# DanHelmy/hdr-realtime-video-pipeline

Hardware: AMD Instinct MI355X
Metric: frames/sec (HDRTVNet++ AGCM+LE+HG fp16 3840x2160 + fused RGB48 post into the pinned host ring); p50 per-frame ms in p50_ms (higher is better)
Workload: dtype f16

## Files before the change

hdr-realtime-video-pipeline_amd/csrc/api_graph.hip:

```cpp
#include "api.h"

namespace hdrtv_host {

void Seq::conv(const std::string &key, const f16 *src0, int c0, const f16 *src1, int c1, int Hi, int Wi, int act, int mode, f16 *dst, int dstC, int Hd, int Wd, const f16 *res1, const f16 *res2, f16 *dst_full, f16 *dst_planar, const f16 *res_planar, const float *dotw, float *dst_dot, int s0_stride)
{
    if (!ok()) return;
    auto it = c->conv.find(key);
    if (it == c->conv.end()) { rc = fail(c, HDRTV_ESTATE, "no packed conv %s", key.c_str()); return; }
    const ConvLayer &L = it->second;
    ConvParams p;
    memset(&p, 0, sizeof p);
    p.src0 = src0; p.src1 = src1; p.c0 = c0; p.c1 = c1;
    p.s0_stride = s0_stride ? s0_stride : c0; p.s1_stride = c1;
    p.Hi = Hi; p.Wi = Wi;
    const int pad = L.ks / 2;
    p.Ho = (Hi + 2 * pad - L.ks) / L.stride + 1;
    p.Wo = (Wi + 2 * pad - L.ks) / L.stride + 1;
    p.wpk = wtp<f16>(c, L.wpk); p.scale = wtp<float>(c, L.scale); p.shift = wtp<float>(c, L.shift);
    p.CoutPad = L.coutPad; p.Cout = L.cout; p.act = act; p.mode = mode;
    p.dst = dst; p.dst_full = dst_full; p.dstC = dstC; p.Hd = Hd; p.Wd = Wd;
    p.res1 = res1; p.res2 = res2; p.dst_planar = dst_planar; p.res_planar = res_planar;
    p.dotw = dotw; p.dst_dot = dst_dot;
    if (c0 + c1 != L.cin) { rc = fail(c, HDRTV_ESTATE, "conv %s: channel mismatch", key.c_str()); return; }
    p.zeros = wtp<f16>(c, c->zeros_off);
// ... 247 lines not shown
            snprintf(b, sizeof b, "cls%d.g", i - 1); ng = wtp<float>(c, c->f32v.at(b));
            snprintf(b, sizeof b, "cls%d.be", i - 1); nb = wtp<float>(c, c->f32v.at(b));
        }
        snprintf(b, sizeof b, "cls%d.w", i);
        const float *w = wtp<float>(c, c->f32v.at(b));
        snprintf(b, sizeof b, "cls%d.b", i);
        const float *bias = wtp<float>(c, c->f32v.at(b));
        int nblk = 0;
        q.chk(cls_block_launch(in, i == 0, cls_ci[i], s.ch[i], s.cw[i], nm, nr, ng, nb, w, bias, cls_co[i], out, s.ch[i + 1],
                               s.cw[i + 1], q.wsp<float>("agcm.part"), q.s, c->cls_q[i].on ? &c->cls_q[i] : nullptr,
                               (i == 4 && c->cls_q[5].on) ? &c->cls_q[5] : nullptr, &nblk),
              "cls_block", c->cls_q[i].on ? "cls_block<fq>" : "cls_block", (double)s.ch[i] * s.cw[i] * cls_ci[i] * cls_co[i]);
        snprintf(a, sizeof a, "agcm.mean%d", i + 1);
        snprintf(b, sizeof b, "agcm.rstd%d", i + 1);
        q.chk(cls_stats_launch(q.wsp<float>("agcm.part"), cls_co[i], nblk, s.ch[i + 1] * s.cw[i + 1], 1e-5f, q.wsp<float>(a),
                               q.wsp<float>(b), q.s),
              "cls_stats", "cls_stats");
    }
    AgcmFoldArgs fa;
    fa.mean5 = q.wsp<float>("agcm.mean5");
    fa.w20 = wtp<float>(c, c->f32v.at("cls20.w")); fa.b20 = wtp<float>(c, c->f32v.at("cls20.b"));
    for (int st = 0; st < 3; ++st) {
        snprintf(a, sizeof a, "gfm.s%d.w", st); fa.ws[st] = wtp<float>(c, c->f32v.at(a));
        snprintf(a, sizeof a, "gfm.s%d.b", st); fa.bs[st] = wtp<float>(c, c->f32v.at(a));
        snprintf(a, sizeof a, "gfm.t%d.w", st); fa.wt[st] = wtp<float>(c, c->f32v.at(a));
        snprintf(a, sizeof a, "gfm.t%d.b", st); fa.bt[st] = wtp<float>(c, c->f32v.at(a));
    }
    fa.w1 = wtp<float>(c, c->f32v.at("agcm.w1")); fa.b1 = wtp<float>(c, c->f32v.at("agcm.b1"));
    fa.w2 = wtp<float>(c, c->f32v.at("agcm.w2")); fa.b2 = wtp<float>(c, c->f32v.at("agcm.b2"));
    fa.w3 = wtp<float>(c, c->f32v.at("agcm.w3")); fa.b3 = wtp<float>(c, c->f32v.at("agcm.b3"));
    if (c->agcm_q8) {
        AgcmFoldQ8Args qa;
        qa.q20 = c->cls_q[5];
        for (int i = 0; i < 6; ++i) qa.qlin[i] = c->lin_q[i];
        qa.P = wtp<float>(c, c->ag_P); qa.Q = wtp<float>(c, c->ag_Q);
        qa.inv2 = c->ag_q[1].inv(); qa.inv3 = c->ag_q[2].inv();
        qa.consts = q.wsp<float>("agcm.qconst");
        q.chk(agcm_fold_q8_launch(fa, qa, q.wsp<float>("agcm.bias"), q.s), "agcm_fold", "agcm_fold<q8>", 128.0 * 6 + 6.0 * (64 + 64 + 3) * 2);
        q.chk(agcm_mlp_q8_launch(rgb, agcm_out, (size_t)c->H * c->W, wtp<int8_t>(c, c->ag_frag), qa.consts, c->ag_q[0].inv(), c->ag_q[0].zoff(),
                                 c->ag_q[1].zoff(), c->ag_q[2].zoff(), q.s),
              "agcm_mlp", "agcm_mlp<q8>", (double)c->H * c->W * (3 * 64 + 64 * 64 + 64 * 3), 12.0 * c->H * c->W);
        return q.rc;
    }
    q.chk(agcm_fold_launch(fa, q.wsp<f16>("agcm.frags"), q.wsp<float>("agcm.bias"), q.s), "agcm_fold", "agcm_fold",
          128.0 * 6 + 6.0 * (64 + 64 + 3) * 2);
    q.chk(agcm_mlp_launch(rgb, agcm_out, (size_t)c->H * c->W, q.wsp<f16>("agcm.frags"), q.wsp<float>("agcm.bias"), q.s),
          "agcm_mlp", "agcm_mlp", (double)c->H * c->W * (3 * 64 + 64 * 64 + 64 * 3), 12.0 * c->H * c->W);
    return q.rc;
}

int run_le(hdrtv_ctx *c, Seq &q, const f16 *img, f16 *out_planar)
{
    const Shapes s = shapes_for(c->H, c->W);
    const int H = s.H, W = s.W;
    f16 *cond = q.wsp<f16>("le.cond");
    f16 *cond1 = q.wsp<f16>("le.cond1"), *cond2 = q.wsp<f16>("le.cond2"), *cond3 = q.wsp<f16>("le.cond3"),
        *cond4 = q.wsp<f16>("le.cond4");
    f16 *h2a = q.wsp<f16>("le.h2a");
    auto qlast = [&](const QLastLayer &Q, QLastArgs &a) -> const QLastArgs * {
        if (!Q.on) return nullptr;
        a.wq = wtp<int8_t>(c, Q.wq); a.ss = wtp<float>(c, Q.ss); a.q_inv = Q.q.inv(); a.q_zoff = Q.q.zoff();
        return &a;
    };
    QLastArgs qa6, qa2;
    if (q.ok() && c->trunk_q8) {
        TrunkQ8Args ta;
        ta.wfrag = wtp<int8_t>(c, c->tq_frag); ta.consts = wtp<float>(c, c->tq_const);
        ta.q1_inv = c->tq_q[0].inv(); ta.q1_zoff = c->tq_q[0].zoff(); ta.q4_inv = c->tq_q[3].inv();
        for (int i = 0; i < 5; ++i) ta.zoff[i] = c->tq_q[i + 1].zoff();
        q.chk(le_cond_trunk_q8_launch(img, H, W, ta, cond, cond1, c->n_cu, q.s), "LE.cond_trunk", "le_cond_trunk_q8",
              (double)H * W * (27 * 64 + 4 * 64 * 64 + 64 * 16), (double)H * W * (6 + 128 + 32));
    } else if (q.ok())
        q.chk(le_cond_trunk_launch(img, H, W, wtp<f16>(c, c->trunk_wfrag), wtp<float>(c, c->trunk_bias), cond, cond1, c->n_cu, q.s,
                                   qlast(c->q_trunk6, qa6)),
              "LE.cond_trunk", c->q_trunk6.on ? "le_cond_trunk<q6>" : "le_cond_trunk", (double)H * W * (27 * 64 + 4 * 64 * 64 + 64 * 16), (double)H * W * (6 + 128 + 32));
    auto isq8 = [&](const char *L) { return c->q8.find(L) != c->q8.end(); };
    auto qof = [&](const char *L) -> const ActQf * { auto it = c->q8.find(L); return it == c->q8.end() ? nullptr : &it->second.q; };
    f16 *h2b = q.wsp<f16>("le.h2b");
    const f16 *a2 = nullptr, *a3 = nullptr, *a4 = nullptr;
    const int8_t *a2q = nullptr, *a3q = nullptr, *a4q = nullptr;
    int astride = 64;
    bool cond2_fused = false;
    if (c->conv.find("LE.CondNet234.0") != c->conv.end()) {
        f16 *x192 = q.wsp<f16>("le.x192");
        cond2_fused = c->var.at("cond2_fused") != 0 && !c->tail_q8 && !c->q_tail2.on;
        if (cond2_fused) { q.tail_w = wtp<f16>(c, c->tail_wfrag); q.tail_b = wtp<float>(c, c->tail_bias); q.tail_out = cond2; }
        q.conv("LE.CondNet234.0", cond, 64, nullptr, 0, H, W, ACT_LRELU01, ST_NHWC, x192, 192, s.H1, s.W1);
        a2 = x192; a3 = x192 + 64; a4 = x192 + 128; astride = 192;
    } else {
        f16 *ca[3] = {q.wsp<f16>("le.c2a"), q.wsp<f16>("le.c3a"), q.wsp<f16>("le.c4a")};
        int8_t *ca8[3] = {q.wsp<int8_t>("le8.c2a"), q.wsp<int8_t>("le8.c3a"), q.wsp<int8_t>("le8.c4a")};
        const char *l0[3] = {"LE.CondNet2.0", "LE.CondNet3.0", "LE.CondNet4.0"}, *l2[3] = {nullptr, "LE.CondNet3.2", "LE.CondNet4.2"};
        const f16 **af[3] = {&a2, &a3, &a4};
        const int8_t **aq[3] = {&a2q, &a3q, &a4q};
        ConvQ8MultiParams mp;
        memset(&mp, 0, sizeof mp);
        mp.src = cond; mp.src_stride = 64; mp.Hi = H; mp.Wi = W; mp.Ho = s.H1; mp.Wo = s.W1;
        double m_macs = 0.0, m_bytes = 2.0 * 64 * H * W;
        for (int i = 0; i < 3; ++i) {
            if (!isq8(l0[i])) continue;
            const QLayer &L = c->q8.at(l0[i]);
            const ActQf *oq = l2[i] ? qof(l2[i]) : (c->tail_q8 ? &c->tl_q[0] : nullptr);
            ConvQ8Group &G = mp.g[mp.ngroups++];
            G.wpk8 = wtp<int8_t>(c, L.wpk8); G.scale = wtp<float>(c, L.scale); G.shift = wtp<float>(c, L.shift);
            G.q_inv = L.q.inv(); G.q_zoff = L.q.zoff(); G.act = ACT_LRELU01;
            G.dst = oq ? (void *)ca8[i] : (void *)ca[i]; G.dst_i8 = oq ? 1 : 0;
            if (oq) { G.oq_inv = oq->inv(); G.oq_zoff = oq->zoff(); *aq[i] = ca8[i]; } else { *af[i] = ca[i]; }
            m_macs += (double)s.H1 * s.W1 * 64 * 9 * 64;
            m_bytes += (double)s.H1 * s.W1 * 64 * (oq ? 1.0 : 2.0) + 9.0 * 64 * 64;
        }
        if (mp.ngroups && q.ok()) {
            char tag[48];
            snprintf(tag, sizeof tag, "conv_q8_multi<%d>", mp.ngroups);
            q.chk(conv_q8_multi_launch(mp, c->n_cu, q.s), "LE.CondNet234.0", tag, m_macs, m_bytes);
        }
        for (int i = 0; i < 3; ++i) {
            if (isq8(l0[i])) {
                continue;
            } else {
                q.conv(l0[i], cond, 64, nullptr, 0, H, W, ACT_LRELU01, ST_NHWC, ca[i], 64, s.H1, s.W1);
                *af[i] = ca[i];
            }
        }
    }
    if (q.ok() && c->tail_q8) {
        if (!a2q) return q.rc = fail(c, HDRTV_ESTATE, "internal: W8A8 CondNet2 tail without int8 input");
        q.chk(cond_tail_q8_launch(a2q, (size_t)s.H1 * s.W1, wtp<int8_t>(c, c->tl_frag), wtp<float>(c, c->tl_const), c->tl_q[1].zoff(), cond2,
                                  c->n_cu, q.s),
              "LE.CondNet2.2+4", "cond_tail_q8", (double)s.H1 * s.W1 * (64 * 64 + 64 * 16), (double)s.H1 * s.W1 * (64 + 32));
    } else if (q.ok() && !cond2_fused)
        q.chk(cond_tail_launch(a2, astride, (size_t)s.H1 * s.W1, wtp<f16>(c, c->tail_wfrag), wtp<float>(c, c->tail_bias), cond2, c->n_cu, q.s,
                               qlast(c->q_tail2, qa2)),
              "LE.CondNet2.2+4", c->q_tail2.on ? "cond_tail<q2>" : "cond_tail", (double)s.H1 * s.W1 * (64 * 64 + 64 * 16), (double)s.H1 * s.W1 * (128 + 32));
    {
        const f16 *af[2] = {a3, a4};
        const int8_t *aq[2] = {a3q, a4q};
        f16 *h2[2] = {h2a, h2b}, *cout[2] = {cond3, cond4};
        const char *l2[2] = {"LE.CondNet3.2", "LE.CondNet4.2"}, *l4[2] = {"LE.CondNet3.4", "LE.CondNet4.4"};
        bool tail4 = false;
        for (int i = 0; i < 2; ++i) {
            const void *h = h2[i];
            bool h_i8 = false;
            if (isq8(l2[i])) {
                const ActQf *oq = qof(l4[i]);
                int8_t *h8 = oq ? q.wsp<int8_t>(i ? "le8.h2b" : "le8.h2a") : nullptr;
                q.convq8(l2[i], aq[i] ? (const void *)aq[i] : (const void *)af[i], aq[i] != nullptr, aq[i] ? 64 : astride, s.H1, s.W1,
                         ACT_LRELU01, oq ? (void *)h8 : (void *)h2[i], 64, oq);
                if (oq) { h = h8; h_i8 = true; }
            } else {
                auto t4 = c->conv.find(l4[i]);
                if (i == 0 && c->var.at("cond3_fused") && !isq8(l4[i]) && t4 != c->conv.end() && t4->second.ks == 1 && t4->second.cin == 64 &&
                    t4->second.cout == 16 && t4->second.coutPad == 32 && t4->second.cin_t == 64) {
                    q.tail_w = wtp<f16>(c, t4->second.wpk); q.tail_s = wtp<float>(c, t4->second.scale); q.tail_b = wtp<float>(c, t4->second.shift);
                    q.tail_out = cout[i];
                    tail4 = true;
                }
                q.conv(l2[i], af[i], 64, nullptr, 0, s.H1, s.W1, ACT_LRELU01, ST_NHWC, h2[i], 64, s.H2, s.W2, nullptr, nullptr, nullptr,
                       nullptr, nullptr, nullptr, nullptr, astride);
            }
            if (tail4) { tail4 = false; continue; }
            if (isq8(l4[i])) q.convq8(l4[i], h, h_i8, 64, s.H2, s.W2, ACT_NONE, cout[i], 16, nullptr);
            else q.conv(l4[i], h2[i], 64, nullptr, 0, s.H2, s.W2, ACT_NONE, ST_NHWC, cout[i], 16, i ? s.H3 : s.H2, i ? s.W3 : s.W2);
        }
    }
    f16 *f0a = q.wsp<f16>("le.f0a"), *f0b = q.wsp<f16>("le.f0b"), *fea0 = q.wsp<f16>("le.fea0"), *up3 = q.wsp<f16>("le.up3");
    bool head_fused = false;
    const bool rows = q.rows_on(H, W, true);
    if (q.ok() && rows && c->var.at("le_rows_i8") && !c->var.at("no_c3q8")) {
        auto qc = c->q8.find("LE.conv_first#c3");
        auto qh = c->q32.find("LE.HR_conv1"), qd = c->q32.find("LE.down_conv1#rows8");
        const SftLayer &S1 = c->sft.at("LE.SFT_layer1");
        if (qc != c->q8.end() && qh != c->q32.end() && qd != c->q32.end() && S1.q && qh->second.coutPad == 32 && qd->second.coutPad == 32) {
            RowsHeadI8Params p;
            memset(&p, 0, sizeof p);
            p.img = img; p.cond = cond1; p.fea0 = fea0; p.fea1 = q.wsp<f16>("le.fea1a"); p.H = H; p.W = W;
            p.cf = q.rows_i8(qc->second); p.hr = q.rows_i8(qh->second); p.dn = q.rows_i8(qd->second); p.s = q.rows_i8(S1);
            p.slope_relu = act_slope(ACT_RELU);
            p.trash = const_cast<char *>(wtp<char>(c, c->dump_off));
            const double npx = (double)H * W;
            q.chk(le_head_rows_i8_launch(p, c->n_cu, q.s), "LE.head", "le_head_rows<i8>",
                  npx * (27.0 * 32 + 2.0 * (16 * 16 + 16 * 32) + 32.0 * 9 * 32 + 32.0 * 9 * 32 / 4), npx * (6 + 32 + 64 + 16) + 2.0 * 9 * 32 * 32);
            head_fused = true;
        }
    }
    if (!head_fused && q.ok() && rows && !c->var.at("no_c3fuse") && !c->var.at("conv32_old")) {
        RowsHeadParams p;
        memset(&p, 0, sizeof p);
        bool qh, qd, qs, qi = isq8("LE.conv_first");
        const ConvLayer *Lh = q.rows_conv("LE.HR_conv1", p.fq_y, qh), *Ld = q.rows_conv("LE.down_conv1", p.fq_f, qd);
        const SftLayer &S1 = c->sft.at("LE.SFT_layer1");
        auto i3 = c->c3.find(qi ? "le.conv_first#fq" : "le.conv_first");
        if (Lh && Ld && q.rows_sft(S1, p.fq_s, qs) && i3 != c->c3.end() && (!qi || c->var.at("le_rows_fq"))) {
            if (qi) p.fq_img = Seq::fqp(c->q8.at("LE.conv_first").q);
            p.fq = (qi ? 1 : 0) | (qh ? 2 : 0) | (qd ? 4 : 0) | (qs ? 8 : 0);
            p.img = img; p.cond = cond1; p.H = H; p.W = W; p.fea0 = fea0; p.fea1 = q.wsp<f16>("le.fea1a");
            p.c3_wfrag = wtp<f16>(c, i3->second.wfrag);
            p.sft_wfrag = wtp<f16>(c, S1.wfrag); p.sft_bias = wtp<float>(c, S1.bias);
            p.w_hr = wtp<f16>(c, Lh->wpk); p.b_hr = wtp<float>(c, Lh->shift); p.w_down = wtp<f16>(c, Ld->wpk); p.b_down = wtp<float>(c, Ld->shift);
            p.trash = const_cast<char *>(wtp<char>(c, c->dump_off));
            p.dump = q.stamp_buf();
            const double npx = (double)H * W;
            q.chk(le_head_rows_launch(p, c->n_cu, q.s), "LE.head", p.fq ? "le_head_rows<fq>" : "le_head_rows",
                  npx * (27.0 * 32 + 2.0 * (16 * 16 + 16 * 32) + 32.0 * 9 * 32 + 32.0 * 9 * 32 / 4), npx * (6 + 32 + 64 + 16) + 2.0 * 2 * 9 * 32 * 32);
            head_fused = true;
        }
    }
    if (!head_fused) {
        if (isq8("LE.conv_first")) {
            if (c->var.at("no_c3q8")) {
                int8_t *img32 = q.wsp<int8_t>("le8.img32");
                const QLayer &Lq = c->q8.at("LE.conv_first");
                if (q.ok()) q.chk(planar3_to_q8_launch(img, (size_t)H * W, Lq.q.inv(), Lq.q.zoff(), img32, q.s), "le.conv_first.pack", "planar3_to_q8", 0.0, 38.0 * H * W);
                q.convq8("LE.conv_first", img32, true, 32, H, W, ACT_RELU, f0a, 32, nullptr);
            } else if (q.ok()) {
                const QLayer &Lq = c->q8.at("LE.conv_first#c3");
                q.chk(conv_c3_q8_launch(img, H, W, wtp<int8_t>(c, Lq.wpk8), wtp<float>(c, Lq.scale), wtp<float>(c, Lq.shift), Lq.q.inv(),
                                        Lq.q.zoff(), ACT_RELU, f0a, c->n_cu, q.s),
                      "LE.conv_first", "conv_c3_q8", (double)H * W * 27 * 32, (double)H * W * (6.0 + 64.0));
            }
            q.conv32("LE.HR_conv1", f0a, cond1, "LE.SFT_layer1", H, W, ACT_RELU, ST_NHWC, fea0, 32, H, W);
        } else {
            const bool fuse = !c->var.at("no_c3fuse") && !c->var.at("conv32_old") && c->q32.find("LE.HR_conv1") == c->q32.end();
            if (fuse) {
                q.conv32("LE.HR_conv1", f0a, cond1, "LE.SFT_layer1", H, W, ACT_RELU, ST_NHWC, fea0, 32, H, W, nullptr, nullptr, nullptr, nullptr,
                         img, "le.conv_first");
            } else {
                q.c3("le.conv_first", img, H, W, ACT_RELU, f0a, nullptr);
                q.conv32("LE.HR_conv1", f0a, cond1, "LE.SFT_layer1", H, W, ACT_RELU, ST_NHWC, fea0, 32, H, W);
            }
        }
    }
    f16 *fea1a = q.wsp<f16>("le.fea1a"), *fea1 = q.wsp<f16>("le.fea1"), *l1b = q.wsp<f16>("le.l1b");
    auto down = [&](const char *key, const f16 *src, int Hi, int Wi, f16 *dst, int Ho, int Wo) {
        if (isq8(key)) q.convq8(key, src, false, 32, Hi, Wi, ACT_RELU, dst, 32, nullptr);
        else q.conv(key, src, 32, nullptr, 0, Hi, Wi, ACT_RELU, ST_NHWC, dst, 32, Ho, Wo);
    };
    if (!head_fused) down("LE.down_conv1", fea0, H, W, fea1a, s.H1, s.W1);
    q.resblock("LE.recon_trunk1.0", fea1a, cond2, s.H1, s.W1, l1b, fea1);
    f16 *fea2a = q.wsp<f16>("le.fea2a"), *fea2 = q.wsp<f16>("le.fea2"), *l2b = q.wsp<f16>("le.l2b");
    down("LE.down_conv2", fea1, s.H1, s.W1, fea2a, s.H2, s.W2);
    q.resblock("LE.recon_trunk2.0", fea2a, cond3, s.H2, s.W2, l2b, fea2);
    f16 *fea3 = q.wsp<f16>("le.fea3"), *l3b = q.wsp<f16>("le.l3b"), *t3x = q.wsp<f16>("le.t3x"), *t3y = q.wsp<f16>("le.t3y");
    down("LE.down_conv3", fea2, s.H2, s.W2, fea3, s.H3, s.W3);
    q.resblock("LE.recon_trunk3.0", fea3, cond4, s.H3, s.W3, l3b, t3x);
    q.resblock("LE.recon_trunk3.1", t3x, cond4, s.H3, s.W3, l3b, t3y);
    q.resblock("LE.recon_trunk3.2", t3y, cond4, s.H3, s.W3, l3b, t3x);
    q.resblock("LE.recon_trunk3.3", t3x, cond4, s.H3, s.W3, l3b, t3y, fea3);
    f16 *up1 = q.wsp<f16>("le.up1"), *t4 = q.wsp<f16>("le.t4");
    q.conv32("LE.up_conv1.0", t3y, nullptr, "", s.H3, s.W3, ACT_RELU, ST_PS, up1, 32, s.H2, s.W2, fea2);
    q.resblock("LE.recon_trunk4.0", up1, cond3, s.H2, s.W2, l2b, t4);
    f16 *up2 = q.wsp<f16>("le.up2"), *t5 = q.wsp<f16>("le.t5");
    q.conv32("LE.up_conv2.0", t4, nullptr, "", s.H2, s.W2, ACT_RELU, ST_PS, up2, 32, s.H1, s.W1, fea1);
    q.resblock("LE.recon_trunk5.0", up2, cond2, s.H1, s.W1, l1b, t5);
    if (q.ok() && rows && c->var.at("le_rows_i8")) {
        auto qu = c->q32.find("LE.up_conv3.0"), qh = c->q32.find("LE.HR_conv2"), ql = c->q32.find("LE.conv_last");
        const SftLayer &S2 = c->sft.at("LE.SFT_layer2");
        if (qu != c->q32.end() && qh != c->q32.end() && ql != c->q32.end() && S2.q && qu->second.coutPad == 128 &&
            qh->second.coutPad == 32 && ql->second.coutPad == 32) {
            RowsTailI8Params p;
            memset(&p, 0, sizeof p);
            p.u = t5; p.fea0 = fea0; p.cond = cond1; p.res_planar = img; p.dst_planar = out_planar; p.H = H; p.W = W;
            p.up = q.rows_i8(qu->second); p.hr = q.rows_i8(qh->second); p.last = q.rows_i8(ql->second); p.s = q.rows_i8(S2);
            p.slope_relu = act_slope(ACT_RELU);
            p.trash = const_cast<char *>(wtp<char>(c, c->dump_off));
            const double npx = (double)H * W;
            q.chk(le_tail_rows_i8_launch(p, c->n_cu, q.s), "LE.tail", "le_tail_rows<i8>",
                  npx * (32.0 * 9 * 128 / 4 + 2.0 * (16 * 16 + 16 * 32) + 32.0 * 9 * 32 + 32.0 * 9 * 3), npx * (16 + 64 + 32 + 6 + 6) + 9.0 * 32 * (128 + 32 + 32));
            return q.rc;
        }
    }
    if (q.ok() && rows) {
        RowsTailParams p;
        memset(&p, 0, sizeof p);
        bool qu, qh, ql, qs;
        const ConvLayer *Lu = q.rows_conv("LE.up_conv3.0", p.fq_u, qu), *Lh = q.rows_conv("LE.HR_conv2", p.fq_y, qh),
                        *Ll = q.rows_conv("LE.conv_last", p.fq_z, ql);
        const SftLayer &S2 = c->sft.at("LE.SFT_layer2");
        if (Lu && Lh && Ll && q.rows_sft(S2, p.fq_s, qs)) {
            p.fq = (qu ? 1 : 0) | (qh ? 2 : 0) | (ql ? 4 : 0) | (qs ? 8 : 0);
            p.u = t5; p.fea0 = fea0; p.cond = cond1; p.res_planar = img; p.dst_planar = out_planar; p.H = H; p.W = W;
            p.w_up = wtp<f16>(c, Lu->wpk); p.b_up = wtp<float>(c, Lu->shift);
            p.sft_wfrag = wtp<f16>(c, S2.wfrag); p.sft_bias = wtp<float>(c, S2.bias);
            p.w_hr = wtp<f16>(c, Lh->wpk); p.b_hr = wtp<float>(c, Lh->shift); p.w_last = wtp<f16>(c, Ll->wpk); p.b_last = wtp<float>(c, Ll->shift);
            p.trash = const_cast<char *>(wtp<char>(c, c->dump_off));
            p.dump = q.stamp_buf();
            const double npx = (double)H * W;
            q.chk(le_tail_rows_launch(p, c->n_cu, q.s), "LE.tail", p.fq ? "le_tail_rows<fq>" : "le_tail_rows",
                  npx * (32.0 * 9 * 128 / 4 + 2.0 * (16 * 16 + 16 * 32) + 32.0 * 9 * 32 + 32.0 * 9 * 3), npx * (16 + 64 + 32 + 6 + 6) + 2.0 * 9 * 32 * (128 + 32 + 32));
            return q.rc;
        }
    }
    q.conv32("LE.up_conv3.0", t5, nullptr, "", s.H1, s.W1, ACT_RELU, ST_PS, up3, 32, H, W, fea0);
    q.conv32("LE.HR_conv2", up3, cond1, "LE.SFT_layer2", H, W, ACT_RELU, ST_NHWC, f0b, 32, H, W);
    q.conv32("LE.conv_last", f0b, nullptr, "", H, W, ACT_NONE, ST_PLANAR3, nullptr, 0, H, W, nullptr, nullptr, out_planar, img);
    return q.rc;
}

size_t hg_need_plan(hdrtv_ctx *c, int Hp, int Wp, HgNeedParams &p)
{
    memset(&p, 0, sizeof p);
    p.Hp = Hp; p.Wp = Wp;
    constexpr int n_layers = (int)(sizeof hg_layers / sizeof hg_layers[0]);
    static_assert(n_layers <= HG_NEED_MAX_LAYERS && n_layers + 2 <= HG_NEED_MAX_TENSORS, "hg_need's tables are too small");
    auto ncell = [&](int level) { return (((Hp >> level) + 15) / 16) * (((Wp >> level) + 15) / 16); };
    const char *names[HG_NEED_MAX_TENSORS];
    int level[HG_NEED_MAX_TENSORS], nt = 0;
    auto tensor = [&](const char *name, int lev) {
        if (!name) name = "part";
        for (int i = 0; i < nt; ++i)
            if (!strcmp(names[i], name)) return i;
        names[nt] = name; level[nt] = lev;
        return nt++;
    };
    for (int i = 0; i < n_layers; ++i) {
        const HgLayer &L = hg_layers[i];
        HgNeedLayer &N = p.L[i];
        N.level = L.level; N.ks = L.ks;
        N.mode = L.mode == ST_POOL ? 1 : (L.ps ? 2 : 0);
        N.in = tensor(L.in, L.level);
        N.skip = L.skip ? tensor(L.skip, L.level) : -1;
        N.out = tensor(L.out, L.out_level());
        N.th = L.ks == 3 && Seq::prw_tile_rows(c, L.mode, L.cout, Hp >> L.level, Wp >> L.level) == 8 ? 8 : 16;
    }
    p.n_layers = n_layers;
    size_t off = 0;
    auto take = [&](size_t bytes) { const size_t o = off; off = (off + bytes + 15) & ~(size_t)15; return (int)o; };
    p.flags_off = take((size_t)ncell(0));
    p.kmap_off = take((size_t)ncell(0));
    p.maps_off = (int)off;
    for (int t = 0; t < nt; ++t) p.map_off[t] = !strcmp(names[t], "part") ? p.flags_off : take((size_t)ncell(level[t]));
    p.maps_bytes = (int)off - p.maps_off;
    for (int i = 0; i < n_layers; ++i) p.L[i].list_off = take(4 * (2 * (size_t)ncell(p.L[i].level) + 4));
    return off;
}

int run_hg(hdrtv_ctx *c, Seq &q, const f16 *base, void *out, int out_f32, bool complete_taps)
{
    const Shapes s = shapes_for(c->H, c->W);
    const int Hp = s.Hp, Wp = s.Wp;
    f16 *img = q.wsp<f16>("hg.img");
    uint8_t *mask = q.wsp<uint8_t>("hg.mask");
    const bool sparse = !complete_taps && c->var.at("hg_sparse") != 0 && !c->hg_i8 && !c->var.at("final_recompute");
    HgNeedParams np;
    if (sparse) {
        hg_need_plan(c, Hp, Wp, np);
        np.base = q.wsp<unsigned char>("hg.need");
    }
    if (q.ws == c->lane_ws[0] && !complete_taps) {
        hipStreamCaptureStatus cap = hipStreamCaptureStatusNone;
        c->taps_partial = sparse;
        c->taps_replayable = sparse && hipStreamIsCapturing(q.s, &cap) == hipSuccess && cap != hipStreamCaptureStatusNone;
        c->taps_stream = q.s;
    }
    if (!complete_taps)
        q.chk(hg_prep_launch(base, s.H, s.W, Hp, Wp, img, mask, c->mask_r, 0.1f, q.s, sparse ? np.base + np.flags_off : nullptr), "hg_prep",
              "hg_prep", 0.0, 13.0 * Hp * Wp);
    if (sparse) q.chk(hg_need_launch(np, q.s), "hg_need", "hg_need", 0.0, 0.0);
    float *part = q.wsp<float>("hg.part");
    const bool light = !c->var.at("final_recompute");
    float *part2 = light ? q.wsp<float>("hg.part2") : nullptr;
    const f16 *w2frag = light ? wtp<f16>(c, c->hgf_wfrag) + 6 * 64 * 8 : nullptr;
    constexpr int n_layers = (int)(sizeof hg_layers / sizeof hg_layers[0]);
    const char *tn[3 * n_layers];
    void *tp[3 * n_layers];
    int nt = 0;
    auto tensor = [&](const char *name) -> void * {
        if (!name) return nullptr;
        for (int i = 0; i < nt; ++i)
            if (!strcmp(tn[i], name)) return tp[i];
        char key[32];
        snprintf(key, sizeof key, "%s%s", c->hg_i8 ? "hg8." : "hg.", name);
        tn[nt] = name;
        tp[nt] = q.wsp<void>(key);
        return tp[nt++];
    };
    q.c3("hg.conv1", img, Hp, Wp, ACT_RELU, nullptr, (f16 *)tensor(hg_layers[0].in), c->hg_q0_inv, c->hg_q0_zero, w2frag, part2);
    char key[32];
    for (const HgLayer &L : hg_layers) {
        snprintf(key, sizeof key, "hg.%s", L.name);
        if (sparse) {
            const HgNeedLayer &N = np.L[&L - hg_layers];
            q.need_list = reinterpret_cast<const int *>(np.base + N.list_off);
            q.need_th = N.th;
            q.need_total = (((Hp >> L.level) + N.th - 1) / N.th) * (((Wp >> L.level) + 15) / 16);
        }
        const int c1 = L.skip_cin, c0 = L.cin - c1, Hi = Hp >> L.level, Wi = Wp >> L.level;
        const int Ho = Hp >> L.out_level(), Wo = Wp >> L.out_level();
        const bool dot3 = L.mode == ST_PS_DOT3;
        const float *dotw = dot3 ? wtp<float>(c, c->hg_w10a) : nullptr;
        float *dst_dot = dot3 ? part : nullptr;
        if (c->hg_i8)
            q.conv8(key, (const int8_t *)tensor(L.in), c0, (const int8_t *)tensor(L.skip), c1, Hi, Wi, L.mode, tensor(L.out), L.out_c(), Ho, Wo, dotw, dst_dot);
        else
            q.conv(key, (const f16 *)tensor(L.in), c0, (const f16 *)tensor(L.skip), c1, Hi, Wi, L.act, L.mode, (f16 *)tensor(L.out), L.out_c(), Ho, Wo,
                   nullptr, nullptr, nullptr, nullptr, nullptr, dotw, dst_dot);
    }
    if (!q.ok() || complete_taps) return q.rc;
    const C3Layer &L1 = c->c3.at("hg.conv1");
    HgFinalFusedArgs fa;
    fa.img = img; fa.mask = mask; fa.part = part; fa.wfrag = wtp<f16>(c, c->hgf_wfrag);
    fa.scale = wtp<float>(c, L1.scale); fa.shift = wtp<float>(c, L1.shift);
    fa.b10 = wtp<float>(c, c->f32v.at("hg.b10"));
    fa.wl = wtp<float>(c, c->f32v.at("hg.wl")); fa.bl = wtp<float>(c, c->f32v.at("hg.bl"));
    fa.out = out; fa.out_f32 = out_f32; fa.H = s.H; fa.W = s.W; fa.Hp = Hp; fa.Wp = Wp;
    if (light)
        q.chk(hg_final_light_launch(fa, part2, q.s), "hg_final", "hg_final_light", (double)s.H * s.W * 6 * 3,
              (double)s.H * s.W * (6 + 1 + 32 + 3 * (out_f32 ? 4 : 2)));
#ifdef HDRTV_AB
    else
        q.chk(hg_final_fused_launch(fa, c->n_cu, q.s), "hg_final", "hg_final_fused", (double)Hp * Wp * (128 * 3 + 6 * 3),
              (double)s.H * s.W * (6 + 1 + 16 + 3 * (out_f32 ? 4 : 2)));
#endif
    return q.rc;
}

}
```

hdr-realtime-video-pipeline_amd/csrc/api_util.hip:

```cpp
#include "api.h"

namespace hdrtv_host {

int fail(hdrtv_ctx *c, int code, const char *fmt, ...)
{
    char buf[512];
    va_list ap;
    va_start(ap, fmt);
    vsnprintf(buf, sizeof buf, fmt, ap);
    va_end(ap);
    if (c) { std::lock_guard<std::mutex> lk(c->err_mu); c->err = buf; }
    return code;
}

namespace {
const std::pair<const char *, int> k_variants[] = {
    {"le_rows", 1},
    {"le_rows_min", 8},
    {"le_rows_i8", 1},
    {"le_rows_fq", 1},
    {"prw", 1},
    {"prw_i8", 1},
    {"pglds_nt_slow", 3},
    {"no_t16", 0},
    {"conv32_old", 0},
    {"conv32_nosplit", 0},
    {"conv32_nw", 0},
    {"no_c3fuse", 0},
    {"no_c3q8", 0},
    {"glds1_old", 0},
    {"hg_sparse", 1},
    {"final_recompute", 0},
    {"cond3_fused", 1},
    {"cond2_fused", 1},
    {"pre_split", 0},
    {"force_ncu", 0},
    {"f32_narrow_below", 0},
    {"f32_mfma", 1},
};
const char *const k_ab_only[] = {"conv32_old", "conv32_nosplit", "conv32_nw", "glds1_old", "final_recompute"};
}
bool variant_allowed(const std::string &name, int value)
{
#ifdef HDRTV_AB
    (void)name; (void)value;
    return true;
#else
    if (value == 0) return true;
    for (const char *n : k_ab_only) if (name == n) return false;
    return true;
#endif
}
void variants_init(hdrtv_ctx *c)
{
    for (const auto &kv : k_variants) c->var[kv.first] = kv.second;
    const char *e = getenv("HDRTV_VARIANTS");
    if (!e) return;
    std::string str(e);
    size_t pos = 0;
    while (pos < str.size()) {
        size_t nx = str.find(',', pos);
        if (nx == std::string::npos) nx = str.size();
        const std::string one = str.substr(pos, nx - pos);
        const size_t eq = one.find('=');
        if (eq != std::string::npos) {
            auto it = c->var.find(one.substr(0, eq));
            if (it != c->var.end() && variant_allowed(it->first, atoi(one.c_str() + eq + 1))) it->second = atoi(one.c_str() + eq + 1);
        }
        pos = nx + 1;
    }
}

}
```

hdr-realtime-video-pipeline_amd/csrc/hg_need.hip:

```cpp
#include "launchers.h"

namespace {

constexpr int NT = 1024;

__device__ __forceinline__ int cells(int n) { return (n + 15) >> 4; }

__global__ __launch_bounds__(NT) void hg_need_kernel(HgNeedParams p)
{
    __shared__ int s_scan[NT];
    const int tid = threadIdx.x;
    for (int i = tid; i < p.maps_bytes; i += NT) p.base[p.maps_off + i] = 0;
    __syncthreads();
    for (int li = p.n_layers - 1; li >= 0; --li) {
        const HgNeedLayer L = p.L[li];
        const int gh = cells(p.Hp >> L.level), gw = cells(p.Wp >> L.level), n = gh * gw;
        const int olev = L.level + (L.mode == 1 ? 1 : 0) - (L.mode == 2 ? 1 : 0);
        const int oh = cells(p.Hp >> olev), ow = cells(p.Wp >> olev);
        const unsigned char *om = p.base + p.map_off[L.out];
        unsigned char *km = p.base + p.kmap_off;
        for (int i = tid; i < n; i += NT) {
            const int y = i / gw, x = i - y * gw;
            int k;
            if (L.mode == 1) {
                k = om[min(y >> 1, oh - 1) * ow + min(x >> 1, ow - 1)];
            } else if (L.mode == 2) {
                k = 0;
                for (int dy = 0; dy < 2; ++dy)
                    for (int dx = 0; dx < 2; ++dx)
                        if (2 * y + dy < oh && 2 * x + dx < ow) k |= om[(2 * y + dy) * ow + 2 * x + dx];
            } else {
                k = om[i];
            }
            km[i] = (unsigned char)(k != 0);
        }
        __syncthreads();
        unsigned char *im = p.base + p.map_off[L.in], *sm = L.skip >= 0 ? p.base + p.map_off[L.skip] : nullptr;
        for (int i = tid; i < n; i += NT) {
            const int y = i / gw, x = i - y * gw;
            int v = km[i];
            if (L.ks == 3 && !v) {
                for (int dy = -1; dy <= 1; ++dy)
                    for (int dx = -1; dx <= 1; ++dx)
                        if ((unsigned)(y + dy) < (unsigned)gh && (unsigned)(x + dx) < (unsigned)gw) v |= km[(y + dy) * gw + x + dx];
            }
            if (v) {
                im[i] = 1;
                if (sm) sm[i] = 1;
            }
        }
        const int per = (n + NT - 1) / NT, c0 = tid * per, c1 = min(n, c0 + per);
        const int ty8 = ((p.Hp >> L.level) + 7) >> 3;
        int cnt = 0;
        for (int i = c0; i < c1; ++i)
            if (km[i]) cnt += (L.th == 8 && 2 * (i / gw) + 1 < ty8) ? 2 : 1;
        s_scan[tid] = cnt;
        __syncthreads();
        for (int d = 1; d < NT; d <<= 1) {
            const int v = tid >= d ? s_scan[tid - d] : 0;
            __syncthreads();
            s_scan[tid] += v;
            __syncthreads();
        }
        int *lst = reinterpret_cast<int *>(p.base + L.list_off);
        int o = s_scan[tid] - cnt;
        if (tid == NT - 1) lst[0] = s_scan[tid];
        for (int i = c0; i < c1; ++i) {
            if (!km[i]) continue;
            const int y = i / gw, x = i - y * gw;
            if (L.th == 8) {
                lst[1 + o++] = 2 * y * gw + x;
                if (2 * y + 1 < ty8) lst[1 + o++] = (2 * y + 1) * gw + x;
            } else {
                lst[1 + o++] = i;
            }
        }
        __syncthreads();
    }
    const int n0 = cells(p.Hp) * cells(p.Wp);
    for (int i = tid; i < n0; i += NT) p.base[p.flags_off + i] = 0;
}

}

hipError_t hg_need_launch(const HgNeedParams &p, hipStream_t s)
{
    if (!p.base || p.n_layers < 1 || p.n_layers > HG_NEED_MAX_LAYERS) return hipErrorInvalidValue;
    hipLaunchKernelGGL(hg_need_kernel, dim3(1), dim3(NT), 0, s, p);
    return hipGetLastError();
}
```

hdr-realtime-video-pipeline_amd/csrc/launchers.h:

```cpp
#pragma once
#include "common.h"

struct DevOnce {
    unsigned char set[64] = {};
    static int cur() { int d = 0; return hipGetDevice(&d) == hipSuccess && d >= 0 && d < 64 ? d : 0; }
    bool need() const { return !set[cur()]; }
    void done() { set[cur()] = 1; }
};

hipError_t conv_igemm_launch(ConvParams p, int cin_t, int bn, int ks, int stride, hipStream_t stream);
hipError_t conv_glds1_launch(ConvParams p, hipStream_t stream, int n_cu = 0, bool old_form = false);
hipError_t conv_pglds_launch(ConvParams p, int n_cu, hipStream_t stream);
hipError_t conv_prw_launch(ConvParams p, int th, int n_cu, hipStream_t stream, bool *list_taken = nullptr);
hipError_t conv_pglds_i8_launch(ConvI8Params p, int n_cu, hipStream_t stream);
hipError_t conv_prw_i8_launch(ConvI8Params p, int th, int n_cu, hipStream_t stream);
hipError_t conv1x1_i8_launch(ConvI8Params p, hipStream_t stream);
hipError_t conv32p_launch(Conv32Params p, int n_cu, hipStream_t stream, int nw = 0);
hipError_t conv32s_launch(Conv32Params p, int n_cu, hipStream_t stream, bool nosplit = false);
hipError_t le_rb_rows_launch(RowsRbParams p, int n_cu, hipStream_t stream);
hipError_t le_rb_rows_i8_launch(RowsRbI8Params p, int n_cu, hipStream_t stream);
hipError_t le_tail_rows_i8_launch(RowsTailI8Params p, int n_cu, hipStream_t stream);
hipError_t le_head_rows_i8_launch(RowsHeadI8Params p, int n_cu, hipStream_t stream);
hipError_t le_tail_rows_launch(RowsTailParams p, int n_cu, hipStream_t stream);
hipError_t le_head_rows_launch(RowsHeadParams p, int n_cu, hipStream_t stream);
hipError_t conv_t16_launch(ConvParams p, hipStream_t stream, int n_cu);
hipError_t conv_q8_launch(ConvQ8Params p, hipStream_t stream, int n_cu);
hipError_t conv_q8_multi_launch(ConvQ8MultiParams p, int n_cu, hipStream_t stream);
hipError_t conv3x3s2_preg_launch(ConvParams p, int n_cu, hipStream_t stream);

hipError_t pre_unpack_launch(const uint8_t *bgr, f16 *out, int H, int W, hipStream_t s);
hipError_t cond_resize_launch(const f16 *in, f16 *out, int H, int W, int Ho, int Wo, const float *wx, const int *xmn,
                              const int *xns, const float *wy, const int *ymn, const int *yns, hipStream_t s);
hipError_t pre_fused_launch(const uint8_t *bgr, f16 *out, f16 *cond, int H, int W, int Ho, int Wo, const float *wx, const int *xmn,
                            const int *xns, const float *wy, const int *ymn, const int *yns, int mode, hipStream_t s);
hipError_t post_u8_launch(const void *in, int is_f32, int H, int W, uint8_t *bgr, hipStream_t s);
hipError_t post_rgb48_launch(const void *in, int is_f32, int H, int W, uint16_t *rgb, int pq, float peak, hipStream_t s,
                             const float *pq_bnd = nullptr);

struct FakeQ { int on; float inv, zoff, scale, zero; };
hipError_t cls_block_launch(const void *in, int in_f16, int Ci, int Hi, int Wi, const float *nmean, const float *nrstd,
                            const float *ngamma, const float *nbeta, const float *Wt, const float *bias, int Co, float *out,
                            int Ho, int Wo, float *part, hipStream_t s, const FakeQ *qin = nullptr, const FakeQ *qstat = nullptr,
                            int *nblk = nullptr);
hipError_t cls_stats_launch(const float *part, int C, int nblk, int n, float eps, float *mean, float *rstd, hipStream_t s);
struct AgcmFoldArgs {
    const float *mean5;
    const float *w20, *b20;
    const float *ws[3], *bs[3], *wt[3], *bt[3];
    const float *w1, *b1, *w2, *b2, *w3, *b3;
};
hipError_t agcm_fold_launch(const AgcmFoldArgs &a, f16 *frags, float *biasbuf, hipStream_t s);
hipError_t agcm_mlp_launch(const f16 *in, f16 *out, size_t npix, const f16 *frags, const float *biasbuf, hipStream_t s);

hipError_t conv_c3_launch(const f16 *in, int H, int W, const f16 *wfrag, const float *scale, const float *shift, int cout,
                          int act, f16 *out, f16 *out_pool, int n_cu, hipStream_t s, float pool_q_inv = 0.f, float pool_q_zero = 0.f,
                          const f16 *w2frag = nullptr, float *part2 = nullptr);
hipError_t conv_c3_q8_launch(const f16 *in, int H, int W, const int8_t *wq, const float *scale, const float *shift, float q_inv,
                             float q_zoff, int act, f16 *out, int n_cu, hipStream_t s);
struct QLastArgs {
    const int8_t *wq;
    const float *ss;
    float q_inv, q_zoff;
};
hipError_t le_cond_trunk_launch(const f16 *img, int H, int W, const f16 *wfrag, const float *bias, f16 *cond, f16 *cond1,
                                int n_cu, hipStream_t s, const QLastArgs *q6 = nullptr);
hipError_t cond_tail_launch(const f16 *x, int x_stride, size_t npx, const f16 *wfrag, const float *bias, f16 *out, int n_cu,
                            hipStream_t s, const QLastArgs *q2 = nullptr);
struct TrunkQ8Args {
    const int8_t *wfrag;
    const float *consts;
    float q1_inv, q1_zoff, q4_inv;
    float zoff[5];
};
hipError_t le_cond_trunk_q8_launch(const f16 *img, int H, int W, const TrunkQ8Args &a, f16 *cond, f16 *cond1, int n_cu, hipStream_t s);
hipError_t cond_tail_q8_launch(const int8_t *x, size_t npx, const int8_t *wfrag, const float *consts, float zoff2, f16 *out, int n_cu,
                               hipStream_t s);
hipError_t agcm_mlp_q8_launch(const f16 *in, f16 *out, size_t npix, const int8_t *wfrag, const float *consts, float q1_inv, float q1_zoff,
                              float zoff2, float zoff3, hipStream_t s);
hipError_t planar3_to_q8_launch(const f16 *in, size_t npix, float inv, float zoff, int8_t *out, hipStream_t s);
struct AgcmFoldQ8Args {
    FakeQ q20, qlin[6];
    const float *P, *Q;
    float inv2, inv3;
    float *consts;
};
hipError_t agcm_fold_q8_launch(const AgcmFoldArgs &a, const AgcmFoldQ8Args &q, float *biasbuf, hipStream_t s);
hipError_t hg_prep_launch(const f16 *base, int H, int W, int Hp, int Wp, f16 *img_pad, uint8_t *mask, float r, float thresh,
                          hipStream_t s, uint8_t *flags = nullptr);
constexpr int HG_NEED_MAX_LAYERS = 24, HG_NEED_MAX_TENSORS = 32;
struct HgNeedLayer {
    int level, mode, ks;
    int in, skip, out;
    int th;
    int list_off;
};
struct HgNeedParams {
    unsigned char *base;
    int Hp, Wp, n_layers;
    int flags_off, maps_off, maps_bytes, kmap_off;
    int map_off[HG_NEED_MAX_TENSORS];
    HgNeedLayer L[HG_NEED_MAX_LAYERS];
};
hipError_t hg_need_launch(const HgNeedParams &p, hipStream_t s);
struct HgFinalFusedArgs {
    const f16 *img;
    const uint8_t *mask;
    const float *part;
    const f16 *wfrag;
    const float *scale, *shift, *b10, *wl, *bl;
    void *out;
    int out_f32, H, W, Hp, Wp;
};
hipError_t hg_final_fused_launch(const HgFinalFusedArgs &a, int n_cu, hipStream_t s);
hipError_t hg_final_light_launch(const HgFinalFusedArgs &a, const float *part2, hipStream_t s);
hipError_t letterbox_launch(const LetterboxParams &p, hipStream_t s);
hipError_t post_scale_launch(const PostScaleParams &p, int is_f32, int pq, hipStream_t s);
hipError_t post_ycbcr10_launch(const Ycbcr10Params &p, int is_f32, int pq, hipStream_t s);
hipError_t rgb48_to_ycbcr10_launch(const Ycbcr10Params &p, hipStream_t s);
hipError_t metrics_launch(const MetricsParams &p, hipStream_t s);
int metrics_blocks(int H, int W);

hipError_t conv_f32_launch(const F32ConvParams &p, int ks, int stride, int n_cu, hipStream_t s);
bool conv_f32_on_mfma(const F32ConvParams &p, int ks, int n_cu);
hipError_t ew_f32_launch(int op, const float *a, const float *b, const float *c, float *y, size_t n, hipStream_t s);
hipError_t avgpool3s2_leaky_f32_launch(const float *x, float *y, int C, int H, int W, float slope, hipStream_t s);
hipError_t instnorm_f32_launch(float *x, const float *gamma, const float *beta, int C, int n, float eps, hipStream_t s);
hipError_t plane_mean_f32_launch(const float *x, float *y, int C, int n, hipStream_t s);
hipError_t gfm_heads_f32_launch(const F32GfmParams &p, hipStream_t s);
hipError_t maxpool2_f32_launch(const float *x, float *y, int C, int H, int W, hipStream_t s);
hipError_t window_f32_launch(const float *x, float *y, int C, int H, int W, int Ho, int Wo, int mode, hipStream_t s);
hipError_t hg_mask_f32_launch(const float *base, float *mask, size_t npix, float r, hipStream_t s);
hipError_t hg_blend_f32_launch(const float *t, const float *img, const float *mask, float *out, int H, int W, int Hp, int Wp,
                               hipStream_t s);
hipError_t pre_f32_launch(const uint8_t *bgr, float *rgb, float *cond, int H, int W, int Ho, int Wo, const float *wx,
                          const int *xmn, const int *xns, const float *wy, const int *ymn, const int *yns, int mode, hipStream_t s);
```

Before: 124.1.

## Rewrite HG sparsity planner with bitmaps, finer need units, LDS chaining, wave scan

Rewrites the single-block hg_need planner so the per-layer need maps are 64-bit bitmaps rather than byte maps. Dilation, pooling and upsampling become word-level bit operations, and maps that chain from one layer to the next stay in LDS. The block-wide scan now uses wave shuffles instead of a barrier-heavy shared-memory loop. The default hg_sparse=2 selects finer need units at deeper levels (down to single pixels), so the tile lists that drive the sparse HG convs become tighter and fewer tiles are scheduled. The cost is more complex bit logic and new validation paths in a kernel that still runs on one block.

```diff
diff --git a/hdr-realtime-video-pipeline_amd/csrc/api_graph.hip b/hdr-realtime-video-pipeline_amd/csrc/api_graph.hip
--- a/hdr-realtime-video-pipeline_amd/csrc/api_graph.hip
+++ b/hdr-realtime-video-pipeline_amd/csrc/api_graph.hip
@@ -573,7 +573,18 @@
     p.Hp = Hp; p.Wp = Wp;
     constexpr int n_layers = (int)(sizeof hg_layers / sizeof hg_layers[0]);
     static_assert(n_layers <= HG_NEED_MAX_LAYERS && n_layers + 2 <= HG_NEED_MAX_TENSORS, "hg_need's tables are too small");
+    constexpr int max_level = [] { int m = 0; for (const HgLayer &L : hg_layers) m = L.level > m ? L.level : m; return m; }();
+    static_assert(max_level < HG_NEED_LEVELS, "hg_need's unit tables have too few levels");
+    memcpy(p.lu, hg_need_unit_log2[c->var.at("hg_sparse") == 1 ? 1 : 2], sizeof p.lu);
     auto ncell = [&](int level) { return (((Hp >> level) + 15) / 16) * (((Wp >> level) + 15) / 16); };
+    auto nwords = [&](int level) {
+        size_t m = 0;
+        for (const auto &tab : hg_need_unit_log2) {
+            const int u = 1 << tab[level], rows = std::max(((Hp >> level) + u - 1) / u, ((Hp >> level) + 7) / 8);
+            m = std::max(m, (size_t)rows * ((((Wp >> level) + u - 1) / u + 63) / 64));
+        }
+        return m;
+    };
     const char *names[HG_NEED_MAX_TENSORS];
     int level[HG_NEED_MAX_TENSORS], nt = 0;
     auto tensor = [&](const char *name, int lev) {
@@ -594,14 +605,33 @@
         N.th = L.ks == 3 && Seq::prw_tile_rows(c, L.mode, L.cout, Hp >> L.level, Wp >> L.level) == 8 ? 8 : 16;
     }
     p.n_layers = n_layers;
+    bool seen[HG_NEED_MAX_TENSORS] = {};
+    for (int i = n_layers - 1; i >= 0; --i) {
+        HgNeedLayer &N = p.L[i];
+        N.in_first = !seen[N.in];
+        seen[N.in] = true;
+        if (N.skip >= 0) { N.skip_first = !seen[N.skip]; seen[N.skip] = true; }
+    }
     size_t off = 0;
     auto take = [&](size_t bytes) { const size_t o = off; off = (off + bytes + 15) & ~(size_t)15; return (int)o; };
     p.flags_off = take((size_t)ncell(0));
-    p.kmap_off = take((size_t)ncell(0));
-    p.maps_off = (int)off;
-    for (int t = 0; t < nt; ++t) p.map_off[t] = !strcmp(names[t], "part") ? p.flags_off : take((size_t)ncell(level[t]));
-    p.maps_bytes = (int)off - p.maps_off;
+    take((size_t)ncell(0));
+    for (int t = 0; t < nt; ++t)
+        if (strcmp(names[t], "part")) take((size_t)ncell(level[t]));
     for (int i = 0; i < n_layers; ++i) p.L[i].list_off = take(4 * (2 * (size_t)ncell(p.L[i].level) + 4));
+    size_t scratch = 0;
+    for (int t = 0; t < nt; ++t) {
+        p.map_off[t] = take(8 * nwords(level[t]));
+        scratch = std::max(scratch, nwords(level[t]));
+        if (!strcmp(names[t], "part")) p.flags_map = t;
+    }
+    for (int i = 0; i < n_layers; ++i) {
+        p.L[i].out_chained = i + 1 < n_layers ? p.L[i + 1].in == p.L[i].out : p.L[i].out == p.flags_map;
+        p.L[i].in_chained = i > 0 && p.L[i - 1].out == p.L[i].in;
+    }
+    p.scratch_words = (int)scratch;
+    p.kbits_off = take(8 * scratch);
+    p.tbits_off = take(8 * scratch);
     return off;
 }
 
diff --git a/hdr-realtime-video-pipeline_amd/csrc/api_util.hip b/hdr-realtime-video-pipeline_amd/csrc/api_util.hip
--- a/hdr-realtime-video-pipeline_amd/csrc/api_util.hip
+++ b/hdr-realtime-video-pipeline_amd/csrc/api_util.hip
@@ -29,7 +29,7 @@
     {"no_c3fuse", 0},
     {"no_c3q8", 0},
     {"glds1_old", 0},
-    {"hg_sparse", 1},
+    {"hg_sparse", 2},
     {"final_recompute", 0},
     {"cond3_fused", 1},
     {"cond2_fused", 1},
diff --git a/hdr-realtime-video-pipeline_amd/csrc/hg_need.hip b/hdr-realtime-video-pipeline_amd/csrc/hg_need.hip
--- a/hdr-realtime-video-pipeline_amd/csrc/hg_need.hip
+++ b/hdr-realtime-video-pipeline_amd/csrc/hg_need.hip
@@ -2,83 +2,158 @@
 
 namespace {
 
-constexpr int NT = 1024;
+constexpr int NT = 1024, LDS_WORDS = 2304;
+using u64 = unsigned long long;
 
-__device__ __forceinline__ int cells(int n) { return (n + 15) >> 4; }
+__constant__ u64 k_tile_bits[5] = {~0ull, 0x5555555555555555ull, 0x1111111111111111ull, 0x0101010101010101ull, 0x0001000100010001ull};
+
+struct Map {
+    int h, w, nw;
+};
+__device__ __forceinline__ Map map_of(const HgNeedParams &p, int level)
+{
+    const int lu = p.lu[level], r = (1 << lu) - 1;
+    Map m;
+    m.h = ((p.Hp >> level) + r) >> lu;
+    m.w = ((p.Wp >> level) + r) >> lu;
+    m.nw = (m.w + 63) >> 6;
+    return m;
+}
+__device__ __forceinline__ u64 word(const u64 *b, const Map &m, int y, int wi)
+{
+    return (unsigned)y < (unsigned)m.h && (unsigned)wi < (unsigned)m.nw ? b[y * m.nw + wi] : 0;
+}
+__device__ __forceinline__ u64 row_mask(int w, int wi)
+{
+    const int n = w - 64 * wi;
+    return n >= 64 ? ~0ull : (n <= 0 ? 0ull : (1ull << n) - 1);
+}
+__device__ __forceinline__ u64 spread2(unsigned v)
+{
+    u64 x = v;
+    x = (x | x << 16) & 0x0000FFFF0000FFFFull;
+    x = (x | x << 8) & 0x00FF00FF00FF00FFull;
+    x = (x | x << 4) & 0x0F0F0F0F0F0F0F0Full;
+    x = (x | x << 2) & 0x3333333333333333ull;
+    x = (x | x << 1) & 0x5555555555555555ull;
+    return x | x << 1;
+}
+__device__ __forceinline__ unsigned pairs_any(u64 v)
+{
+    u64 x = (v | v >> 1) & 0x5555555555555555ull;
+    x = (x | x >> 1) & 0x3333333333333333ull;
+    x = (x | x >> 2) & 0x0F0F0F0F0F0F0F0Full;
+    x = (x | x >> 4) & 0x00FF00FF00FF00FFull;
+    x = (x | x >> 8) & 0x0000FFFF0000FFFFull;
+    x = (x | x >> 16) & 0x00000000FFFFFFFFull;
+    return (unsigned)x;
+}
 
 __global__ __launch_bounds__(NT) void hg_need_kernel(HgNeedParams p)
 {
-    __shared__ int s_scan[NT];
+    __shared__ u64 s_k[LDS_WORDS], s_t[LDS_WORDS], s_n[LDS_WORDS];
+    __shared__ int s_wave[NT / 64];
     const int tid = threadIdx.x;
-    for (int i = tid; i < p.maps_bytes; i += NT) p.base[p.maps_off + i] = 0;
+    {
+        const Map m = map_of(p, 0);
+        const HgNeedLayer &L = p.L[p.n_layers - 1];
+        u64 *fb = L.out_chained && m.h * m.nw <= LDS_WORDS ? s_n : reinterpret_cast<u64 *>(p.base + p.map_off[p.flags_map]);
+        unsigned char *fl = p.base + p.flags_off;
+        constexpr int NW = NT / 64, B = 8;
+        const int lane = tid & 63, n0 = m.h * m.nw;
+        for (int i0 = tid >> 6; i0 < n0; i0 += B * NW) {
+            int at[B];
+            unsigned char c[B];
+#pragma unroll
+            for (int j = 0; j < B; ++j) {
+                const int i = i0 + j * NW, y = i / m.nw, x = 64 * (i - y * m.nw) + lane;
+                at[j] = i < n0 && x < m.w ? y * m.w + x : -1;
+                c[j] = at[j] >= 0 ? fl[at[j]] : 0;
+            }
+#pragma unroll
+            for (int j = 0; j < B; ++j) {
+                const u64 v = __ballot(c[j] != 0);
+                if (at[j] >= 0) fl[at[j]] = 0;
+                if (lane == 0 && i0 + j * NW < n0) fb[i0 + j * NW] = v;
+            }
+        }
+    }
     __syncthreads();
     for (int li = p.n_layers - 1; li >= 0; --li) {
         const HgNeedLayer L = p.L[li];
-        const int gh = cells(p.Hp >> L.level), gw = cells(p.Wp >> L.level), n = gh * gw;
         const int olev = L.level + (L.mode == 1 ? 1 : 0) - (L.mode == 2 ? 1 : 0);
-        const int oh = cells(p.Hp >> olev), ow = cells(p.Wp >> olev);
-        const unsigned char *om = p.base + p.map_off[L.out];
-        unsigned char *km = p.base + p.kmap_off;
-        for (int i = tid; i < n; i += NT) {
-            const int y = i / gw, x = i - y * gw;
-            int k;
-            if (L.mode == 1) {
-                k = om[min(y >> 1, oh - 1) * ow + min(x >> 1, ow - 1)];
-            } else if (L.mode == 2) {
+        const Map mk = map_of(p, L.level), mo = map_of(p, olev);
+        const int lu = p.lu[L.level], nk = mk.h * mk.nw;
+        const int sh = p.lu[olev] - lu + olev - L.level;
+        const int lth = L.th == 8 ? 3 : 4, lbw = 4 - lu;
+        const int ty_n = ((p.Hp >> L.level) + L.th - 1) >> lth, tx_n = ((p.Wp >> L.level) + 15) >> 4, nt = ty_n * mk.nw;
+        const bool lds = max(nk, nt) <= LDS_WORDS;
+        u64 *km = lds ? s_k : reinterpret_cast<u64 *>(p.base + p.kbits_off);
+        u64 *tm = lds ? s_t : reinterpret_cast<u64 *>(p.base + p.tbits_off);
+        const u64 *om = L.out_chained && mo.h * mo.nw <= LDS_WORDS ? s_n : reinterpret_cast<const u64 *>(p.base + p.map_off[L.out]);
+        for (int i = tid; i < nk; i += NT) {
+            const int y = i / mk.nw, wi = i - y * mk.nw;
+            u64 k;
+            if (sh == 0) {
+                k = word(om, mo, y, wi);
+            } else if (sh > 0) {
+                k = spread2((unsigned)(word(om, mo, y >> 1, wi >> 1) >> (32 * (wi & 1))));
+            } else {
                 k = 0;
                 for (int dy = 0; dy < 2; ++dy)
-                    for (int dx = 0; dx < 2; ++dx)
-                        if (2 * y + dy < oh && 2 * x + dx < ow) k |= om[(2 * y + dy) * ow + 2 * x + dx];
-            } else {
-                k = om[i];
+                    k |= (u64)pairs_any(word(om, mo, 2 * y + dy, 2 * wi)) | (u64)pairs_any(word(om, mo, 2 * y + dy, 2 * wi + 1)) << 32;
             }
-            km[i] = (unsigned char)(k != 0);
+            km[i] = k & row_mask(mk.w, wi);
         }
         __syncthreads();
-        unsigned char *im = p.base + p.map_off[L.in], *sm = L.skip >= 0 ? p.base + p.map_off[L.skip] : nullptr;
-        for (int i = tid; i < n; i += NT) {
-            const int y = i / gw, x = i - y * gw;
-            int v = km[i];
-            if (L.ks == 3 && !v) {
-                for (int dy = -1; dy <= 1; ++dy)
-                    for (int dx = -1; dx <= 1; ++dx)
-                        if ((unsigned)(y + dy) < (unsigned)gh && (unsigned)(x + dx) < (unsigned)gw) v |= km[(y + dy) * gw + x + dx];
+        u64 *ig = reinterpret_cast<u64 *>(p.base + p.map_off[L.in]), *im = L.in_chained && nk <= LDS_WORDS ? s_n : ig;
+        u64 *sm = L.skip >= 0 ? reinterpret_cast<u64 *>(p.base + p.map_off[L.skip]) : nullptr;
+        for (int i = tid; i < nk; i += NT) {
+            const int y = i / mk.nw, wi = i - y * mk.nw;
+            u64 v = km[i];
+            if (L.ks == 3) {
+                for (int dy = -1; dy <= 1; ++dy) {
+                    const u64 c = word(km, mk, y + dy, wi);
+                    v |= c | c << 1 | c >> 1 | word(km, mk, y + dy, wi - 1) >> 63 | word(km, mk, y + dy, wi + 1) << 63;
+                }
+                v &= row_mask(mk.w, wi);
             }
-            if (v) {
-                im[i] = 1;
-                if (sm) sm[i] = 1;
-            }
+            im[i] = L.in_first ? v : (ig[i] | v);
+            if (sm) sm[i] = L.skip_first ? v : (sm[i] | v);
         }
-        const int per = (n + NT - 1) / NT, c0 = tid * per, c1 = min(n, c0 + per);
-        const int ty8 = ((p.Hp >> L.level) + 7) >> 3;
+        const int r_sh = lth - lu;
+        for (int i = tid; i < nt; i += NT) {
+            const int ty = i / mk.nw, wi = i - ty * mk.nw;
+            const int r0 = r_sh >= 0 ? ty << r_sh : ty >> -r_sh, nr = r_sh >= 0 ? 1 << r_sh : 1;
+            u64 v = 0;
+            for (int r = r0; r < min(r0 + nr, mk.h); ++r) v |= km[r * mk.nw + wi];
+            for (int s = 1; s < (1 << lbw); s <<= 1) v |= v >> s;
+            tm[i] = v & k_tile_bits[lbw];
+        }
+        __syncthreads();
+        const int per = (nt + NT - 1) / NT, c0 = tid * per, c1 = min(nt, c0 + per);
         int cnt = 0;
-        for (int i = c0; i < c1; ++i)
-            if (km[i]) cnt += (L.th == 8 && 2 * (i / gw) + 1 < ty8) ? 2 : 1;
-        s_scan[tid] = cnt;
+        for (int i = c0; i < c1; ++i) cnt += __popcll(tm[i]);
+        int incl = cnt;
+        for (int d = 1; d < 64; d <<= 1) {
+            const int v = __shfl_up(incl, d, 64);
+            if ((tid & 63) >= d) incl += v;
+        }
+        if ((tid & 63) == 63) s_wave[tid >> 6] = incl;
         __syncthreads();
-        for (int d = 1; d < NT; d <<= 1) {
-            const int v = tid >= d ? s_scan[tid - d] : 0;
-            __syncthreads();
-            s_scan[tid] += v;
-            __syncthreads();
+        int o = incl - cnt, total = 0;
+        for (int w = 0; w < NT / 64; ++w) {
+            const int v = s_wave[w];
+            if (w < (tid >> 6)) o += v;
+            total += v;
         }
         int *lst = reinterpret_cast<int *>(p.base + L.list_off);
-        int o = s_scan[tid] - cnt;
-        if (tid == NT - 1) lst[0] = s_scan[tid];
+        if (tid == 0) lst[0] = total;
         for (int i = c0; i < c1; ++i) {
-            if (!km[i]) continue;
-            const int y = i / gw, x = i - y * gw;
-            if (L.th == 8) {
-                lst[1 + o++] = 2 * y * gw + x;
-                if (2 * y + 1 < ty8) lst[1 + o++] = (2 * y + 1) * gw + x;
-            } else {
-                lst[1 + o++] = i;
-            }
+            const int ty = i / mk.nw, wi = i - ty * mk.nw;
+            for (u64 v = tm[i]; v; v &= v - 1) lst[1 + o++] = ty * tx_n + ((64 * wi + __ffsll(v) - 1) >> lbw);
         }
-        __syncthreads();
     }
-    const int n0 = cells(p.Hp) * cells(p.Wp);
-    for (int i = tid; i < n0; i += NT) p.base[p.flags_off + i] = 0;
 }
 
 }
@@ -86,6 +161,14 @@
 hipError_t hg_need_launch(const HgNeedParams &p, hipStream_t s)
 {
     if (!p.base || p.n_layers < 1 || p.n_layers > HG_NEED_MAX_LAYERS) return hipErrorInvalidValue;
+    for (int i = 0; i < p.n_layers; ++i) {
+        const HgNeedLayer &L = p.L[i];
+        const int olev = L.level + (L.mode == 1 ? 1 : 0) - (L.mode == 2 ? 1 : 0);
+        if (L.level < 0 || L.level >= HG_NEED_LEVELS || olev < 0 || olev >= HG_NEED_LEVELS) return hipErrorInvalidValue;
+        const int sh = p.lu[olev] - p.lu[L.level] + olev - L.level;
+        if (p.lu[L.level] < 0 || p.lu[L.level] > 4 || sh < -1 || sh > 1 || (L.th != 8 && L.th != 16)) return hipErrorInvalidValue;
+    }
+    if (p.lu[0] != 4) return hipErrorInvalidValue;
     hipLaunchKernelGGL(hg_need_kernel, dim3(1), dim3(NT), 0, s, p);
     return hipGetLastError();
 }
diff --git a/hdr-realtime-video-pipeline_amd/csrc/launchers.h b/hdr-realtime-video-pipeline_amd/csrc/launchers.h
--- a/hdr-realtime-video-pipeline_amd/csrc/launchers.h
+++ b/hdr-realtime-video-pipeline_amd/csrc/launchers.h
@@ -87,17 +87,24 @@
 hipError_t agcm_fold_q8_launch(const AgcmFoldArgs &a, const AgcmFoldQ8Args &q, float *biasbuf, hipStream_t s);
 hipError_t hg_prep_launch(const f16 *base, int H, int W, int Hp, int Wp, f16 *img_pad, uint8_t *mask, float r, float thresh,
                           hipStream_t s, uint8_t *flags = nullptr);
-constexpr int HG_NEED_MAX_LAYERS = 24, HG_NEED_MAX_TENSORS = 32;
+constexpr int HG_NEED_MAX_LAYERS = 24, HG_NEED_MAX_TENSORS = 32, HG_NEED_LEVELS = 6;
+constexpr int hg_need_unit_log2[3][HG_NEED_LEVELS] = {{4, 4, 4, 4, 4, 4}, {4, 4, 4, 4, 4, 4}, {4, 2, 1, 0, 0, 0}};
 struct HgNeedLayer {
     int level, mode, ks;
     int in, skip, out;
+    int in_first, skip_first;
+    int out_chained;
+    int in_chained;
     int th;
     int list_off;
 };
 struct HgNeedParams {
     unsigned char *base;
     int Hp, Wp, n_layers;
-    int flags_off, maps_off, maps_bytes, kmap_off;
+    int lu[HG_NEED_LEVELS];
+    int flags_off;
+    int flags_map;
+    int kbits_off, tbits_off, scratch_words;
     int map_off[HG_NEED_MAX_TENSORS];
     HgNeedLayer L[HG_NEED_MAX_LAYERS];
 };
```

After: 137.5, median of 6. 1.11x the previous value.
